# distributed-information-bottleneck/distributed-information-bottleneck.github.io

Measured on AMD Instinct MI355X. Metric: DIB train samples/sec (fwd+KL+bwd+Adam), higher is better.
Workload: dtype f32

## Files before the change

distributed-information-bottleneck.github.io_amd/csrc/dib_fused.h:

```cpp
#pragma once
#include "dib_common.h"
#include "dib_gemm.h"

struct DibFusedFwdArgs {
  const float* P;
  const int* row_idx; long long row0; int batch;
  const float* params;
  const long long* w_off;
  const long long* b_off;
  const int4* featmap;
  int n_blocks;
  int act;
  float* h1; float* h2; float* enc_out; float* U; float* kl_partial;
  unsigned long long* h2mask;
  unsigned long long* h1mask;
  int F; unsigned long long seed; unsigned step; int deterministic;
  const unsigned* step_dev;
};

template <int H1, int H2, int E>
struct DibFusedCfg {
  static constexpr int E2 = 2 * E;
  static constexpr int N3 = (E2 + 31) / 32 * 32;
  static constexpr int K1P = 36;
  static constexpr int P2 = H1 + 4, P3 = H2 + 4;
  static constexpr int W1_FLOATS = H1 * K1P, W2_FLOATS = H2 * P2, W3_FLOATS = N3 * P3;
  static constexpr int B_FLOATS = H1 + H2 + N3;
  static constexpr int PATCH = 32 * 36;
  static constexpr int LDS_FLOATS = W1_FLOATS + W2_FLOATS + W3_FLOATS + B_FLOATS + 8 * PATCH;
  static constexpr int T1 = H1 / 32, T2 = H2 / 32, T3 = N3 / 32;
};

typedef float dib_nt4 __attribute__((ext_vector_type(4)));

__device__ __forceinline__ int dib_crow(int r, int h) { return (r & 3) + 8 * (r >> 2) + 4 * h; }

__device__ __forceinline__ float dib_sigma(float lv) {
  return __builtin_amdgcn_exp2f(0.72134752044448170f * lv);
}

__device__ __forceinline__ float dib_neg_slope(int act) { return act == 1 ? 0.f : (act == 2 ? 0.2f : (act == 7 ? 0.1f : 1.f)); }
template <bool RELU>
__device__ __forceinline__ void dib_act_tile(float slope, dib_f32x16& v) {
#pragma unroll
  for (int r = 0; r < 16; ++r) v[r] = RELU ? fmaxf(v[r], 0.f) : fmaxf(v[r], 0.f) + slope * fminf(v[r], 0.f);
}

__device__ __forceinline__ int dib_patch_row(int lane, int pss) {
  return (lane >> 4) + 8 * ((lane >> 3) & 1) + 4 * (pss & 1) + 16 * (pss >> 1);
}

__device__ __forceinline__ int dib_store_idx(int lane) {
  return 4 * (((lane & 31) >> 2) >> 1) + (lane & 3);
}
__device__ __forceinline__ int dib_store_col(int lane) { return (dib_store_idx(lane) & 7) * 4; }
__device__ __forceinline__ int dib_store_row(int lane, int pss) {
  const int q = (lane & 31) >> 2;
  const int G = 2 * (lane >> 5) + ((0x96 >> q) & 1);
  return G + 4 * (pss & 1) + 16 * (pss >> 1) + 8 * (dib_store_idx(lane) >> 3);
}

__device__ __forceinline__ void dib_store_tile(float* __restrict__ patch, const dib_f32x16& c, float* __restrict__ dst,
                                               long long ld, int rows_valid, int lane) {
  const int m = lane & 31, h = lane >> 5;
#pragma unroll
  for (int g = 0; g < 4; ++g)
    *reinterpret_cast<float4*>(patch + m * 36 + 8 * g + 4 * h) = make_float4(c[4 * g], c[4 * g + 1], c[4 * g + 2], c[4 * g + 3]);
  __builtin_amdgcn_wave_barrier();
  const int cc = dib_store_col(lane);
  const int r0 = dib_store_row(lane, 0);
  const float* src = patch + r0 * 36 + cc;
  float4 v[4];
#pragma unroll
  for (int pss = 0; pss < 4; ++pss) v[pss] = *reinterpret_cast<const float4*>(src + (4 * (pss & 1) + 16 * (pss >> 1)) * 36);
  __builtin_amdgcn_wave_barrier();
  float* out = dst + (long long)r0 * ld + cc;
  if (rows_valid >= 32) {
#pragma unroll
    for (int pss = 0; pss < 4; ++pss)
      __builtin_nontemporal_store(dib_nt4{v[pss].x, v[pss].y, v[pss].z, v[pss].w},
                                  reinterpret_cast<dib_nt4*>(out + (long long)(4 * (pss & 1) + 16 * (pss >> 1)) * ld));
  } else {
#pragma unroll
    for (int pss = 0; pss < 4; ++pss)
      if (r0 + 4 * (pss & 1) + 16 * (pss >> 1) < rows_valid)
        *reinterpret_cast<float4*>(out + (long long)(4 * (pss & 1) + 16 * (pss >> 1)) * ld) = v[pss];
  }
}

template <int COUNT, typename LoadF, typename StoreF>
__device__ __forceinline__ void dib_stage_batched(int tid, LoadF load, StoreF store) {
  constexpr int ITERS = (COUNT + 511) / 512;
#pragma unroll
  for (int it0 = 0; it0 < ITERS; it0 += 8) {
    float v[8];
#pragma unroll
    for (int u = 0; u < 8; ++u) {
      const int i = tid + (it0 + u) * 512;
      v[u] = (it0 + u < ITERS && i < COUNT) ? load(i) : 0.f;
    }
#pragma unroll
    for (int u = 0; u < 8; ++u) {
      const int i = tid + (it0 + u) * 512;
      if (it0 + u < ITERS && i < COUNT) store(i, v[u]);
    }
  }
}

#ifdef DIB_FUSED_TIMING
__device__ long long dib_fused_dbg[16];
#define DIB_FT(i) do { __builtin_amdgcn_sched_barrier(0); const long long now_ = clock64(); tacc_[i] += now_ - tprev_; tprev_ = now_; \
                       __builtin_amdgcn_sched_barrier(0); } while (0)
#else
#define DIB_FT(i) do { } while (0)
#endif

template <int T>
__device__ __forceinline__ unsigned long long dib_sign_bits(const dib_f32x16 (&t)[T]) {
  static_assert(T <= 4, "one 64-bit mask word per lane");
  unsigned int word[2] = {0u, 0u};
#pragma unroll
  for (int w = 0; w < (T + 1) / 2; ++w)
#pragma unroll
    for (int idx = (16 * T - 32 * w - 1 < 31 ? 16 * T - 32 * w - 1 : 31); idx >= 0; --idx) {
      const int e = 32 * w + idx;
      int on;
      asm("v_med3_i32 %0, %1, 0, 1" : "=v"(on) : "v"(t[e >> 4][e & 15]));
      asm("v_lshl_or_b32 %0, %1, 1, %2" : "=v"(word[w]) : "v"(word[w]), "v"(on));
    }
  return ((unsigned long long)word[1] << 32) | word[0];
}
template <bool RELU>
__device__ __forceinline__ void dib_mask_tile(dib_f32x16& acc, unsigned long long bits, int jo, float slope) {
  const unsigned int word = (unsigned int)(bits >> (32 * ((16 * jo) >> 5)));
#pragma unroll
  for (int r = 0; r < 16; ++r) {
    const int keep = __builtin_amdgcn_sbfe(word, (16 * jo + r) & 31, 1);
    acc[r] = RELU ? __int_as_float(__float_as_int(acc[r]) & keep) : acc[r] * (keep ? 1.f : slope);
  }
}

template <int H1, int H2, int E, bool RELU>
__global__ void __launch_bounds__(512)
dib_fused_encoder_fwd_kernel(DibFusedFwdArgs a) {
  using C = DibFusedCfg<H1, H2, E>;
  extern __shared__ __attribute__((aligned(16))) float lds[];
  float* Wt1 = lds;
  float* Wt2 = Wt1 + C::W1_FLOATS;
  float* Wt3 = Wt2 + C::W2_FLOATS;
  float* Bs = Wt3 + C::W3_FLOATS;
  float* patch = Bs + C::B_FLOATS + (threadIdx.x >> 6) * C::PATCH;

  const int f = blockIdx.y;
  const int tid = threadIdx.x, lane = tid & 63, wave = tid >> 6;
  const int m = lane & 31, h = lane >> 5;
  const int4 fm = a.featmap[f];
  const int in_dim = fm.y;
  const int F = a.F;
  const float* Pf = a.P + (long long)fm.w * a.batch;

  {
    const float* W1 = a.params + a.w_off[0 * F + f];
    const float* W2 = a.params + a.w_off[1 * F + f];
    const float* W3 = a.params + a.w_off[2 * F + f];
    const float* b1 = a.params + a.b_off[0 * F + f];
    const float* b2 = a.params + a.b_off[1 * F + f];
    const float* b3 = a.params + a.b_off[2 * F + f];
    dib_stage_batched<H1 * 32>(tid, [&](int i) { const int k = i / H1; return (k < in_dim) ? W1[i] : 0.f; },
                               [&](int i, float v) { const int k = i / H1, n = i - k * H1; Wt1[n * C::K1P + k] = v; });
    dib_stage_batched<H1 * H2>(tid, [&](int i) { return W2[i]; },
                               [&](int i, float v) { const int k = i / H2, n = i - k * H2; Wt2[n * C::P2 + k] = v; });
    dib_stage_batched<H2 * C::N3>(tid, [&](int i) { const int k = i / C::N3, n = i - k * C::N3;
                                                    return (n < C::E2) ? W3[(long long)k * C::E2 + n] : 0.f; },
                                  [&](int i, float v) { const int k = i / C::N3, n = i - k * C::N3; Wt3[n * C::P3 + k] = v; });
    for (int i = tid; i < H1; i += 512) Bs[i] = b1[i];
    for (int i = tid; i < H2; i += 512) Bs[H1 + i] = b2[i];
    for (int i = tid; i < C::N3; i += 512) Bs[H1 + H2 + i] = (i < C::E2) ? b3[i] : 0.f;
  }
  __syncthreads();

  const int n_tiles = (a.batch + 255) / 256;
  const unsigned nstep = a.step_dev ? a.step_dev[0] : a.step;
  const float slope = dib_neg_slope(a.act);
  const int ksteps1 = 4 * ((in_dim + 7) / 8);
  float kl_acc = 0.f;

  auto load_p = [&](int tile, float (&dstp)[8]) {
    const int bb = min(tile * 256 + wave * 32 + m, a.batch - 1);
    const float* src = Pf + (long long)bb * in_dim;
#pragma unroll
    for (int r = 0; r < 8; ++r) {
      const int k = dib_crow(r, h);
      const float v = src[min(k, in_dim - 1)];
      dstp[r] = (k < in_dim) ? v : 0.f;
    }
  };
  float p[8], pn[8];
  if ((int)blockIdx.x < n_tiles) load_p(blockIdx.x, p);

#ifdef DIB_FUSED_TIMING
  long long tacc_[9] = {0, 0, 0, 0, 0, 0, 0, 0, 0};
  long long tprev_ = clock64();
  const long long tstart_ = tprev_;
  const long long wstart_ = wall_clock64();
  int ntl_ = 0;
#endif
  for (int tile = blockIdx.x; tile < n_tiles; tile += gridDim.x) {
#ifdef DIB_FUSED_TIMING
    ++ntl_;
#endif
    const int wrow0 = tile * 256 + wave * 32;
    const int rows_valid = min(32, a.batch - wrow0);
    const int b = wrow0 + m;
    const bool valid = b < a.batch;
    const long long grow = a.row_idx ? (long long)a.row_idx[valid ? b : 0] : a.row0 + b;
    {
      const int nt = tile + gridDim.x;
      load_p(nt < n_tiles ? nt : tile, pn);
    }

    dib_f32x16 h1[C::T1];
#pragma unroll
    for (int jo = 0; jo < C::T1; ++jo) {
      dib_f32x16 acc;
#pragma unroll
      for (int r = 0; r < 16; ++r) acc[r] = Bs[32 * jo + dib_crow(r, h)];
#pragma unroll
      for (int g = 0; g < 2; ++g) {
        if (4 * g < ksteps1) {
          const float4 w = *reinterpret_cast<const float4*>(Wt1 + (32 * jo + m) * C::K1P + 8 * g + 4 * h);
          acc = DIB_MFMA(w.x, p[4 * g + 0], acc);
          acc = DIB_MFMA(w.y, p[4 * g + 1], acc);
          acc = DIB_MFMA(w.z, p[4 * g + 2], acc);
          acc = DIB_MFMA(w.w, p[4 * g + 3], acc);
        }
      }
      dib_act_tile<RELU>(slope, acc);
      h1[jo] = acc;
    }
    DIB_FT(0);
    if (a.h1 != nullptr) {
      float* dst = a.h1 + ((long long)f * a.batch + wrow0) * H1;
#pragma unroll
      for (int jo = 0; jo < C::T1; ++jo) dib_store_tile(patch, h1[jo], dst + 32 * jo, H1, rows_valid, lane);
    }
    if (a.h1mask != nullptr && valid) a.h1mask[((long long)f * a.batch + b) * 2 + h] = dib_sign_bits<C::T1>(h1);
    DIB_FT(1);
    dib_f32x16 h2[C::T2];
    if constexpr (C::T2 % 2 == 0) {
#pragma unroll
    for (int jo = 0; jo < C::T2; jo += 2) {
      dib_f32x16 acc0, acc1;
#pragma unroll
      for (int r = 0; r < 16; ++r) { acc0[r] = Bs[H1 + 32 * jo + dib_crow(r, h)]; acc1[r] = Bs[H1 + 32 * jo + 32 + dib_crow(r, h)]; }
      const float* w0p = Wt2 + (32 * jo + m) * C::P2 + 4 * h;
      const float* w1p = w0p + 32 * C::P2;
      float4 wa = *reinterpret_cast<const float4*>(w0p), wb = *reinterpret_cast<const float4*>(w1p);
#pragma unroll
      for (int st = 0; st < 4 * C::T1; ++st) {
        const int ji = st >> 2, g = st & 3, sn = st + 1 < 4 * C::T1 ? st + 1 : st;
        const float4 wan = *reinterpret_cast<const float4*>(w0p + 8 * sn), wbn = *reinterpret_cast<const float4*>(w1p + 8 * sn);
        __builtin_amdgcn_sched_barrier(0);
        acc0 = DIB_MFMA(wa.x, h1[ji][4 * g + 0], acc0);
// ... 58 lines not shown
        const float4 wan = *reinterpret_cast<const float4*>(w0p + 8 * sn), wbn = *reinterpret_cast<const float4*>(w1p + 8 * sn);
        __builtin_amdgcn_sched_barrier(0);
        acc0 = DIB_MFMA(wa.x, h2[ji][4 * g + 0], acc0);
        acc1 = DIB_MFMA(wb.x, h2[ji][4 * g + 0], acc1);
        acc0 = DIB_MFMA(wa.y, h2[ji][4 * g + 1], acc0);
        acc1 = DIB_MFMA(wb.y, h2[ji][4 * g + 1], acc1);
        acc0 = DIB_MFMA(wa.z, h2[ji][4 * g + 2], acc0);
        acc1 = DIB_MFMA(wb.z, h2[ji][4 * g + 2], acc1);
        acc0 = DIB_MFMA(wa.w, h2[ji][4 * g + 3], acc0);
        acc1 = DIB_MFMA(wb.w, h2[ji][4 * g + 3], acc1);
        asm volatile("" : "+v"(acc0));
        asm volatile("" : "+v"(acc1));
        __builtin_amdgcn_sched_barrier(0);
        wa = wan; wb = wbn;
      }
      o[0] = acc0;
      o[1] = acc1;
    } else {
#pragma unroll
    for (int jo = 0; jo < C::T3; ++jo) {
      dib_f32x16 acc;
#pragma unroll
      for (int r = 0; r < 16; ++r) acc[r] = Bs[H1 + H2 + 32 * jo + dib_crow(r, h)];
#pragma unroll
      for (int ji = 0; ji < C::T2; ++ji) {
#pragma unroll
        for (int g = 0; g < 4; ++g) {
          const float4 w = *reinterpret_cast<const float4*>(Wt3 + (32 * jo + m) * C::P3 + 32 * ji + 8 * g + 4 * h);
          acc = DIB_MFMA(w.x, h2[ji][4 * g + 0], acc);
          acc = DIB_MFMA(w.y, h2[ji][4 * g + 1], acc);
          acc = DIB_MFMA(w.z, h2[ji][4 * g + 2], acc);
          acc = DIB_MFMA(w.w, h2[ji][4 * g + 3], acc);
        }
      }
      o[jo] = acc;
    }
    }
    DIB_FT(5);
    float klp = 0.f;
    float* eo = a.enc_out + ((long long)f * a.batch + b) * C::E2;
    float* up = a.U + (long long)b * ((long long)F * E) + (long long)f * E;
    constexpr int NG = E / 8;
    dib_f32x16 ut[(E >= 32) ? (E / 32) : 1];
#pragma unroll
    for (int gi = 0; gi < NG; ++gi) {
      const int t_mu = (E >= 32) ? (gi >> 2) : 0;
      const int g_mu = (E >= 32) ? (gi & 3) : gi;
      const int t_lv = (E >= 32) ? (t_mu + E / 32) : 0;
      const int g_lv = (E >= 32) ? g_mu : (gi + E / 8);
      const int e0 = 32 * t_mu + 8 * g_mu + 4 * h;
      float eps[4] = {0.f, 0.f, 0.f, 0.f};
      if (!a.deterministic) dib_eps4(a.seed, nstep, (uint32_t)grow, (uint32_t)f, (uint32_t)(e0 >> 2), eps);
      float4 mu = make_float4(o[t_mu][4 * g_mu], o[t_mu][4 * g_mu + 1], o[t_mu][4 * g_mu + 2], o[t_mu][4 * g_mu + 3]);
      float4 lv = make_float4(o[t_lv][4 * g_lv], o[t_lv][4 * g_lv + 1], o[t_lv][4 * g_lv + 2], o[t_lv][4 * g_lv + 3]);
      float4 u;
      const float4 sg = make_float4(dib_sigma(lv.x), dib_sigma(lv.y), dib_sigma(lv.z), dib_sigma(lv.w));
      u.x = mu.x + sg.x * eps[0];
      u.y = mu.y + sg.y * eps[1];
      u.z = mu.z + sg.z * eps[2];
      u.w = mu.w + sg.w * eps[3];
      ut[t_mu][4 * g_mu] = u.x; ut[t_mu][4 * g_mu + 1] = u.y; ut[t_mu][4 * g_mu + 2] = u.z; ut[t_mu][4 * g_mu + 3] = u.w;
      if (valid) {
        if (E < 32) {
          *reinterpret_cast<float4*>(eo + e0) = mu;
          *reinterpret_cast<float4*>(eo + E + e0) = lv;
          *reinterpret_cast<float4*>(up + e0) = u;
        }
        klp += 0.5f * ((mu.x * mu.x + sg.x * sg.x - lv.x - 1.f) + (mu.y * mu.y + sg.y * sg.y - lv.y - 1.f) +
                       (mu.z * mu.z + sg.z * sg.z - lv.z - 1.f) + (mu.w * mu.w + sg.w * sg.w - lv.w - 1.f));
      }
    }
    DIB_FT(6);
    if (E >= 32) {
      float* eo_w = a.enc_out + ((long long)f * a.batch + wrow0) * C::E2;
#pragma unroll
      for (int jo = 0; jo < C::T3; ++jo) dib_store_tile(patch, o[jo], eo_w + 32 * jo, C::E2, rows_valid, lane);
      float* u_w = a.U + (long long)wrow0 * ((long long)F * E) + (long long)f * E;
#pragma unroll
      for (int jo = 0; jo < ((E >= 32) ? (E / 32) : 1); ++jo)
        dib_store_tile(patch, ut[jo], u_w + 32 * jo, (long long)F * E, rows_valid, lane);
    }
    DIB_FT(7);
    kl_acc += dib_wave_sum(klp);
#pragma unroll
    for (int r = 0; r < 8; ++r) p[r] = pn[r];
    DIB_FT(8);
  }
#ifdef DIB_FUSED_TIMING
  if (blockIdx.x == 0 && blockIdx.y == 0 && tid == 0) {
    for (int i = 0; i < 9; ++i) dib_fused_dbg[i] = tacc_[i];
    dib_fused_dbg[9] = clock64() - tstart_;
    dib_fused_dbg[10] = ntl_;
    dib_fused_dbg[11] = wall_clock64() - wstart_;
  }
#endif
  if (lane == 0) a.kl_partial[((long long)blockIdx.x * 8 + wave) * F + f] = kl_acc;
}

typedef float dib_f32x4 __attribute__((ext_vector_type(4)));
#define DIB_MFMA16(a, b, c) __builtin_amdgcn_mfma_f32_16x16x4f32((a), (b), (c), 0, 0, 0)

struct DibFusedBwdArgs {
  const float* P; int batch;
  const float* params; const long long* w_off; const long long* b_off; const int4* featmap;
  int act;
  const unsigned long long* h1mask; const unsigned long long* h2mask;
  const float* enc_out; const float* U; const float* GU;
  float* dout; float* dh2;
  float* dw1_partial;
  const float* beta_dev; float inv_bg;
  int F;
};

template <int H1, int H2, int E>
struct DibFusedBwdCfg {
  static constexpr int E2 = 2 * E;
  static constexpr int N3 = (E2 + 31) / 32 * 32;
  static constexpr int P2 = H2 + 4, P3 = N3 + 4;
  static constexpr int W2_FLOATS = H1 * P2, W3_FLOATS = H2 * P3;
  static constexpr int PATCH = 32 * 36;
  static constexpr int LDS_FLOATS = W2_FLOATS + W3_FLOATS + 8 * PATCH;
  static constexpr int T1 = H1 / 32, T2 = H2 / 32, T3 = N3 / 32;
};

struct DibTile4 { float4 a, b, c, d; };
__device__ __forceinline__ DibTile4 dib_tile_gload(const float* __restrict__ src, long long ld, int rows_valid, int lane) {
  const int cc = (lane & 7) * 4;
  DibTile4 t;
  auto ld4 = [&](int pss) {
    const dib_nt4 v = __builtin_nontemporal_load(reinterpret_cast<const dib_nt4*>(src + (long long)min(dib_patch_row(lane, pss), rows_valid - 1) * ld + cc));
    return make_float4(v.x, v.y, v.z, v.w);
  };
  t.a = ld4(0); t.b = ld4(1); t.c = ld4(2); t.d = ld4(3);
  return t;
}
__device__ __forceinline__ dib_f32x16 dib_tile_to_frag(float* __restrict__ patch, const DibTile4 t, int lane) {
  const int cc = (lane & 7) * 4, m = lane & 31, h = lane >> 5;
  *reinterpret_cast<float4*>(patch + dib_patch_row(lane, 0) * 36 + cc) = t.a;
  *reinterpret_cast<float4*>(patch + dib_patch_row(lane, 1) * 36 + cc) = t.b;
  *reinterpret_cast<float4*>(patch + dib_patch_row(lane, 2) * 36 + cc) = t.c;
  *reinterpret_cast<float4*>(patch + dib_patch_row(lane, 3) * 36 + cc) = t.d;
  __builtin_amdgcn_wave_barrier();
  const float4 q0 = *reinterpret_cast<const float4*>(patch + m * 36 + 4 * h);
  const float4 q1 = *reinterpret_cast<const float4*>(patch + m * 36 + 8 + 4 * h);
  const float4 q2 = *reinterpret_cast<const float4*>(patch + m * 36 + 16 + 4 * h);
  const float4 q3 = *reinterpret_cast<const float4*>(patch + m * 36 + 24 + 4 * h);
  __builtin_amdgcn_wave_barrier();
  dib_f32x16 c;
  c[0] = q0.x; c[1] = q0.y; c[2] = q0.z; c[3] = q0.w; c[4] = q1.x; c[5] = q1.y; c[6] = q1.z; c[7] = q1.w;
  c[8] = q2.x; c[9] = q2.y; c[10] = q2.z; c[11] = q2.w; c[12] = q3.x; c[13] = q3.y; c[14] = q3.z; c[15] = q3.w;
  return c;
}

__device__ __forceinline__ int dib_dw1_row(int s8, int lg) { return s8 + 8 * lg; }

template <int H1, int H2, int E, bool RELU>
__global__ void __launch_bounds__(512)
dib_fused_encoder_bwd_kernel(DibFusedBwdArgs a) {
  static_assert(E % 32 == 0, "fused backward: embedding dimension must be a multiple of 32");
  static_assert(H1 / 32 <= 4 && H2 / 32 <= 4, "act' bit masks: one 64-bit word per (lane, layer)");
  using C = DibFusedBwdCfg<H1, H2, E>;
  extern __shared__ __attribute__((aligned(16))) float lds[];
  float* W2i = lds;
  float* W3i = W2i + C::W2_FLOATS;
  float* patch = W3i + C::W3_FLOATS + (threadIdx.x >> 6) * C::PATCH;

  const int f = blockIdx.y;
  const int tid = threadIdx.x, lane = tid & 63, wave = tid >> 6;
  const int m = lane & 31, h = lane >> 5;
  const int4 fm = a.featmap[f];
  const int in_dim = fm.y;
  const int F = a.F;
  const float* Pf = a.P + (long long)fm.w * a.batch;
  {
    const float* W2 = a.params + a.w_off[1 * F + f];
    const float* W3 = a.params + a.w_off[2 * F + f];
    dib_stage_batched<H1 * H2>(tid, [&](int i) { return W2[i]; },
                               [&](int i, float v) { const int k1 = i / H2, k2 = i - k1 * H2; W2i[k1 * C::P2 + k2] = v; });
    dib_stage_batched<H2 * C::N3>(tid, [&](int i) { const int k2 = i / C::N3, n = i - k2 * C::N3;
                                                    return (n < C::E2) ? W3[(long long)k2 * C::E2 + n] : 0.f; },
                                  [&](int i, float v) { const int k2 = i / C::N3, n = i - k2 * C::N3; W3i[k2 * C::P3 + n] = v; });
  }
  __syncthreads();

  const int n_tiles = (a.batch + 255) / 256;
  const float slope = dib_neg_slope(a.act);
  const float kb = a.beta_dev[0] * a.inv_bg;
  dib_f32x4 dw1[2 * C::T1];
#pragma unroll
  for (int t = 0; t < 2 * C::T1; ++t) dw1[t] = dib_f32x4{0.f, 0.f, 0.f, 0.f};
  const int l15 = lane & 15, lg = lane >> 4;

  for (int tile = blockIdx.x; tile < n_tiles; tile += gridDim.x) {
    const int wrow0 = tile * 256 + wave * 32;
    if (wrow0 >= a.batch) continue;
    const int rows_valid = min(32, a.batch - wrow0);
    const int b = min(wrow0 + m, a.batch - 1);
    const unsigned long long hbits = a.h2mask[((long long)f * a.batch + b) * 2 + h];
    const unsigned long long h1bits = a.h1mask[((long long)f * a.batch + b) * 2 + h];
    dib_f32x16 dout[C::T3];
    {
      const float* eo = a.enc_out + ((long long)f * a.batch + wrow0) * C::E2;
      const long long so = (long long)wrow0 * ((long long)F * E) + (long long)f * E;
#pragma unroll
      for (int t = 0; t < E / 32; ++t) {
        const DibTile4 vm = dib_tile_gload(eo + 32 * t, C::E2, rows_valid, lane);
        const DibTile4 vl = dib_tile_gload(eo + E + 32 * t, C::E2, rows_valid, lane);
        const DibTile4 vg = dib_tile_gload(a.GU + so + 32 * t, (long long)F * E, rows_valid, lane);
        const DibTile4 vu = dib_tile_gload(a.U + so + 32 * t, (long long)F * E, rows_valid, lane);
        const dib_f32x16 mu = dib_tile_to_frag(patch, vm, lane);
        const dib_f32x16 lv = dib_tile_to_frag(patch, vl, lane);
        const dib_f32x16 g = dib_tile_to_frag(patch, vg, lane);
        const dib_f32x16 u = dib_tile_to_frag(patch, vu, lane);
#pragma unroll
        for (int r = 0; r < 16; ++r) {
          const float s = dib_sigma(lv[r]);
          dout[t][r] = g[r] + kb * mu[r];
          dout[t + E / 32][r] = g[r] * (u[r] - mu[r]) * 0.5f + kb * 0.5f * (s * s - 1.f);
        }
      }
      float* dd = a.dout + ((long long)f * a.batch + wrow0) * C::E2;
#pragma unroll
      for (int t = 0; t < C::T3; ++t) dib_store_tile(patch, dout[t], dd + 32 * t, C::E2, rows_valid, lane);
    }

    float pa[8];
#pragma unroll
    for (int s8 = 0; s8 < 8; ++s8) {
      const int rl = dib_dw1_row(s8, lg);
      const float v = Pf[(long long)min(wrow0 + rl, a.batch - 1) * in_dim + min(l15, in_dim - 1)];
      pa[s8] = (rl < rows_valid) ? (l15 < in_dim ? v : (l15 == in_dim ? 1.f : 0.f)) : 0.f;
    }

    dib_f32x16 dh2[C::T2];
    {
      float* dg = a.dh2 + ((long long)f * a.batch + wrow0) * H2;
#pragma unroll
      for (int jo = 0; jo < C::T2; ++jo) {
        dib_f32x16 acc;
#pragma unroll
        for (int r = 0; r < 16; ++r) acc[r] = 0.f;
#pragma unroll
        for (int jt = 0; jt < C::T3; ++jt)
#pragma unroll
          for (int g = 0; g < 4; ++g) {
            const float4 w = *reinterpret_cast<const float4*>(W3i + (32 * jo + m) * C::P3 + 32 * jt + 8 * g + 4 * h);
            acc = DIB_MFMA(w.x, dout[jt][4 * g + 0], acc);
            acc = DIB_MFMA(w.y, dout[jt][4 * g + 1], acc);
            acc = DIB_MFMA(w.z, dout[jt][4 * g + 2], acc);
            acc = DIB_MFMA(w.w, dout[jt][4 * g + 3], acc);
          }
        dib_mask_tile<RELU>(acc, hbits, jo, slope);
        dh2[jo] = acc;
        dib_store_tile(patch, acc, dg + 32 * jo, H2, rows_valid, lane);
      }
    }

    {
#pragma unroll
      for (int jo = 0; jo < C::T1; ++jo) {
        dib_f32x16 acc;
#pragma unroll
        for (int r = 0; r < 16; ++r) acc[r] = 0.f;
#pragma unroll
        for (int jt = 0; jt < C::T2; ++jt)
#pragma unroll
          for (int g = 0; g < 4; ++g) {
            const float4 w = *reinterpret_cast<const float4*>(W2i + (32 * jo + m) * C::P2 + 32 * jt + 8 * g + 4 * h);
            acc = DIB_MFMA(w.x, dh2[jt][4 * g + 0], acc);
            acc = DIB_MFMA(w.y, dh2[jt][4 * g + 1], acc);
            acc = DIB_MFMA(w.z, dh2[jt][4 * g + 2], acc);
            acc = DIB_MFMA(w.w, dh2[jt][4 * g + 3], acc);
          }
        dib_mask_tile<RELU>(acc, h1bits, jo, slope);
#pragma unroll
        for (int g = 0; g < 4; ++g)
          *reinterpret_cast<float4*>(patch + m * 36 + 8 * g + 4 * h) =
              make_float4(acc[4 * g], acc[4 * g + 1], acc[4 * g + 2], acc[4 * g + 3]);
        __builtin_amdgcn_wave_barrier();
#pragma unroll
        for (int s8 = 0; s8 < 8; ++s8) {
          const int rl = dib_dw1_row(s8, lg);
          const float2 bb = *reinterpret_cast<const float2*>(patch + rl * 36 + 2 * l15);
          dw1[2 * jo] = DIB_MFMA16(pa[s8], bb.x, dw1[2 * jo]);
          dw1[2 * jo + 1] = DIB_MFMA16(pa[s8], bb.y, dw1[2 * jo + 1]);
        }
        __builtin_amdgcn_wave_barrier();
      }
    }
  }
  {
    float* dst = a.dw1_partial + (((long long)blockIdx.x * 8 + wave) * F + f) * (16ll * H1);
#pragma unroll
    for (int t = 0; t < 2 * C::T1; ++t)
#pragma unroll
      for (int r = 0; r < 4; ++r) {
        const int n = 32 * (t >> 1) + 2 * l15 + (t & 1);
        dst[(long long)(lg * 4 + r) * H1 + n] = dw1[t][r];
      }
  }
}

__global__ void __launch_bounds__(256)
dib_dw1_reduce_kernel(const float* __restrict__ partial, int nparts, int F, int H1, const long long* __restrict__ w_off,
                      const long long* __restrict__ b_off, const int4* __restrict__ featmap, float* __restrict__ grads) {
  const int f = blockIdx.x, k = blockIdx.y;
  const int in_dim = featmap[f].y;
  if (k > in_dim) return;
  const long long pstride = (long long)F * 16 * H1;
  for (int n = threadIdx.x; n < H1; n += 256) {
    const float* src = partial + ((long long)f * 16 + k) * H1 + n;
    float s = 0.f;
    int pz = 0;
    for (; pz + 8 <= nparts; pz += 8) {
      float v[8];
#pragma unroll
      for (int u = 0; u < 8; ++u) v[u] = src[(pz + u) * pstride];
#pragma unroll
      for (int u = 0; u < 8; ++u) s += v[u];
    }
    for (; pz < nparts; ++pz) s += src[pz * pstride];
    if (k < in_dim) grads[w_off[f] + (long long)k * H1 + n] = s;
    else grads[b_off[f] + n] = s;
  }
}
```

distributed-information-bottleneck.github.io_amd/csrc/host/encoder.h:

```cpp

template <int H1, int H2, int E, bool RELU>
static int launch_fused_fwd(const DibFusedFwdArgs& a, int gx, int F, hipStream_t st) {
  using C = DibFusedCfg<H1, H2, E>;
  const size_t lds = (size_t)C::LDS_FLOATS * sizeof(float);
  return launch_lds<&dib_fused_encoder_fwd_kernel<H1, H2, E, RELU>>(dim3(gx, F), dim3(512), lds, st, a);
}

static int fused_gx(const dib_layout* l, int batch) { return std::max(1, std::min(cdiv(batch, 256), std::max(1, 256 / l->F))); }

static bool fused_bwd_ok(const dib_layout* l) {
  if (!(l->fused_id == 0 || l->fused_id == 1)) return false;
  for (int f = 0; f < l->F; ++f)
    if (l->in_dim[f] > 15) return false;
  return true;
}

static bool use_small_enc(const dib_layout* l, int batch);
static dib_layout::H1Plan h1_recompute_plan(const dib_layout* l, const dib_layout::WsMap& m, const float* w, int batch) {
  dib_layout::H1Plan r;
  if (!knobs().wgrad_recompute_h1 || l->fused_id != 0 || !fused_bwd_ok(l) || l->h1_side.empty() || !l->dev_h1_side) return r;
  if (use_small_enc(l, batch)) return r;
  const GemmCall& c = l->enc_wgrad[1];
  WgradStreamPlan sp;
  if (!wgrad_stream_plan(l->table.data() + c.first, c, w + m.enc_h[0], w + m.g_enc_h[1], batch, m.nsplit, m.rows_per_split,
// ... 149 lines not shown
  float* w = (float*)ws;
  float* gt = wgrad_target(m, w, grads);
  const long long sstride = align_up(l->n_params, 4);
  int rc = DIB_OK;
  const bool small = use_small_enc(l, batch);
  const bool fused = small || fused_bwd_ok(l);
  const int LE = l->n_enc + 1;
  if (stages & 1) {
    if (small) {
      rc = small_encoder_bwd(l, m, w, batch, params, beta_dev, inv_global_batch, st);
    } else if (fused) {
      rc = fused_encoder_bwd(l, m, w, batch, params, beta_dev, inv_global_batch, st);
    } else {
      { ProfScope ps(kProfOther, (hipStream_t)stream);
      DIB_LAUNCH(dib_reparam_kl_bwd_kernel, dim3(m.kl_blocks, l->F), dim3(256), 0, st, w + m.enc_out, w + m.g_u,
                         w + m.U, w + m.dout, beta_dev, inv_global_batch, batch, l->F, l->E); }
      rc = (int)hipGetLastError();
    }
    if (rc) return rc;
  }
  for (int ly = LE - 1; ly >= 0; --ly) {
    const bool last = ly == LE - 1;
    const float* gout = last ? w + m.dout : w + m.g_enc_h[ly];
    const float* hin = ly == 0 ? w + m.P : w + m.enc_h[ly - 1];
    const bool wgrad_here = (last ? (stages & 2) : (stages & 1)) && !(fused && ly == 0);
    if (wgrad_here && ly == 1 && fused && !small) {
      const dib_layout::H1Plan plan = h1_plan_of(l, ws);
      if (plan.recompute) {
        const GemmCall& c = l->enc_wgrad[ly];
        rc = launch_wgrad_h1(plan.ch, l->act == 1, l->dev_groups, l->dev_h1_side, c, w + m.P, params, gout, gt, gt, batch, plan.nsplit,
                             plan.rows_per_split, sstride, st);
        if (rc == DIB_OK && m.nsplit > 1)
          rc = retire_stale_slabs(l, batch, l->table.data() + c.first, c.count, plan.nsplit, m.nsplit, gt, sstride, st);
        if (rc) return rc;
        continue;
      }
    }
    if (wgrad_here) {
      const bool halve = l->enc_wgrad[ly].max_n <= 64 && m.nsplit >= 32 && (m.nsplit % 2) == 0;
      rc = launch_gemm<2>(l, l->enc_wgrad[ly], hin, gout, gt, nullptr, nullptr, gt, batch, 0,
                          halve ? m.nsplit / 2 : m.nsplit, halve ? 2 * m.rows_per_split : m.rows_per_split, sstride, st,
                          m.nsplit);
      if (rc) return rc;
    }
    if ((stages & 1) && ly >= 1 && !fused) {
      rc = launch_gemm<1>(l, l->enc_dgrad[ly], gout, params, w + m.g_enc_h[ly - 1], nullptr, hin, nullptr, batch,
                          l->act, 1, 0, 0, st);
      if (rc) return rc;
    }
  }
  return DIB_OK;
}

extern "C" {

int dib_encoder_bank_fwd(dib_layout* l, const float* x, int64_t ldx, const int32_t* row_idx, int64_t row0, int batch,
                         const float* params, uint64_t seed, uint32_t step, int deterministic, void* ws,
                         dib_stream_t stream) {
  if (!l || !x || !params || !ws || batch <= 0) return DIB_E_ARG;
  if (!l->dev_groups) return DIB_E_WORKSPACE;
  hipStream_t st = (hipStream_t)stream;
  const auto m = l->map(batch);
  float* w = (float*)ws;
  { std::lock_guard<std::mutex> lk(l->wg_mu); l->fwd_training[ws] = !(deterministic & DIB_FWD_INFERENCE); }
  if (use_small_enc(l, batch)) {
    if (!(deterministic & DIB_FWD_INFERENCE)) h1_plan_record(l, ws, dib_layout::H1Plan());
    int rc = small_encoder_fwd(l, m, w, x, ldx, row_idx, row0, batch, params, seed, step, deterministic, st);
    if (rc || (deterministic & DIB_FWD_DEFER_SUMS)) return rc;
    ProfScope ps(kProfOther, st);
    DIB_LAUNCH(dib_colsum_partials_kernel, dim3(l->F), dim3(256), 0, st, w + m.kl_partial, small_tiles(batch), l->F,
                       w + m.step_out);
    return (int)hipGetLastError();
  }
  { ProfScope ps(kProfOther, (hipStream_t)stream);
  if ((long long)cdiv(l->sum_d, 64) * cdiv(batch, 64) >= 512)
    DIB_LAUNCH(dib_posenc_kernel<64>, dim3(cdiv(l->sum_d, 64), cdiv(batch, 64)), dim3(256), 0, st, x, (long long)ldx,
                       (const int*)row_idx, (long long)row0, batch, l->dev_colmap, l->sum_d, l->n_blocks, w + m.P);
  else
    DIB_LAUNCH(dib_posenc_kernel<16>, dim3(cdiv(l->sum_d, 64), cdiv(batch, 16)), dim3(256), 0, st, x, (long long)ldx,
                       (const int*)row_idx, (long long)row0, batch, l->dev_colmap, l->sum_d, l->n_blocks, w + m.P); }
  int rc = (int)hipGetLastError();
  if (rc) return rc;
  if (l->fused_id >= 0) {
    int gx = 1;
    rc = fused_encoder_fwd(l, m, w, x, ldx, row_idx, row0, batch, params, seed, step, deterministic, st, &gx);
    if (rc) return rc;
    if (deterministic & DIB_FWD_DEFER_SUMS) return DIB_OK;
    { ProfScope ps(kProfOther, (hipStream_t)stream);
    DIB_LAUNCH(dib_colsum_partials_kernel, dim3(l->F), dim3(256), 0, st, w + m.kl_partial, gx * 8, l->F,
                       w + m.step_out); }
    return (int)hipGetLastError();
  }
  rc = encoder_chain_fwd(l, m, w, batch, params, 0, l->F, st);
  if (rc) return rc;
  { ProfScope ps(kProfOther, (hipStream_t)stream);
  DIB_LAUNCH(dib_reparam_kl_fwd_kernel, dim3(m.kl_blocks, l->F), dim3(256), 0, st, w + m.enc_out, w + m.U,
                     w + m.kl_partial, (const int*)row_idx, (long long)row0, batch, l->F, l->E,
                     (unsigned long long)seed, (unsigned)step, deterministic & DIB_FWD_DETERMINISTIC, l->step_dev); }
  rc = (int)hipGetLastError();
  if (rc) return rc;
  if (deterministic & DIB_FWD_DEFER_SUMS) return DIB_OK;
  { ProfScope ps(kProfOther, (hipStream_t)stream);
  DIB_LAUNCH(dib_colsum_partials_kernel, dim3(l->F), dim3(256), 0, st, w + m.kl_partial, m.kl_blocks, l->F,
                     w + m.step_out); }
  return (int)hipGetLastError();
}

int dib_encoder_bank_bwd(dib_layout* l, int batch, const float* params, float* grads, const float* beta_dev,
                         float inv_global_batch, void* ws, dib_stream_t stream) {
  return encoder_bank_bwd_stages(l, batch, params, grads, beta_dev, inv_global_batch, 3, ws, stream);
}

int dib_encoder_bank_bwd_stage(dib_layout* l, int batch, const float* params, float* grads, const float* beta_dev,
                               float inv_global_batch, int stage, void* ws, dib_stream_t stream) {
  if (stage != 1 && stage != 2) return DIB_E_ARG;
  return encoder_bank_bwd_stages(l, batch, params, grads, beta_dev, inv_global_batch, stage, ws, stream);
}

int dib_workspace_h1_materialize(dib_layout* l, int batch, const float* params, void* ws, dib_stream_t stream) {
  if (!l || !params || !ws || batch <= 0 || l->n_enc < 1) return DIB_E_ARG;
  if (!l->dev_groups) return DIB_E_WORKSPACE;
  const auto m = l->map(batch);
  float* w = (float*)ws;
  return launch_gemm<0>(l, l->enc_fwd[0], w + m.P, params, w + m.enc_h[0], params, nullptr, nullptr, batch, l->act, 1, 0, 0,
                        (hipStream_t)stream);
}

int dib_encode_deterministic(dib_layout* l, int feature, const float* x_f, int n, const float* params, float* out,
                             void* ws, dib_stream_t stream) {
  if (!l || !x_f || !params || !out || !ws || n <= 0) return DIB_E_ARG;
  if (feature < 0 || feature >= l->F) return DIB_E_ARG;
  if (!l->dev_groups) return DIB_E_WORKSPACE;
  hipStream_t st = (hipStream_t)stream;
  const auto m = l->map(n);
  float* w = (float*)ws;
  const int d = l->dims[feature];
  { ProfScope ps(kProfOther, (hipStream_t)stream);
  DIB_LAUNCH(dib_posenc_kernel<64>, dim3(cdiv(d, 64), cdiv(n, 64)), dim3(256), 0, st, x_f, (long long)d,
                     (const int*)nullptr, 0ll, n, l->dev_colmap + l->x_off[feature], d, l->n_blocks, w + m.P); }
  int rc = (int)hipGetLastError();
  if (rc) return rc;
  rc = encoder_chain_fwd(l, m, w, n, params, feature, 1, st);
  if (rc) return rc;
  const int w2 = 2 * l->E;
  return (int)hipMemcpyAsync(out, w + m.enc_out + (int64_t)feature * n * w2, (size_t)n * w2 * sizeof(float),
                             hipMemcpyDeviceToDevice, st);
}

#ifdef DIB_FUSED_TIMING
int dib_fused_debug_read(long long* out16) {
  if (hipDeviceSynchronize() != hipSuccess) return DIB_E_ARG;
  return (int)hipMemcpyFromSymbol(out16, HIP_SYMBOL(dib_fused_dbg), 16 * sizeof(long long));
}
#endif

}
```

Measured before the change: 8.870 million.

## Prefetch next tile inputs and pair MFMA chains in fused encoder backward

Restructures the fused encoder backward loop so the next tile's masks, P values, GU/U and enc_out tiles are loaded into registers during the current tile's GEMMs (a software pipeline). The dout elementwise math is now done in row-major form before the LDS transpose, and dout is written with direct non-temporal global stores instead of going through the LDS patch. The dh2 and dh1 GEMMs process two output tiles at a time with double-buffered LDS weight reads and sched barriers. It also adds timing instrumentation behind a compile flag. The prefetch raises register pressure and may lower occupancy or cause spills.

```diff
diff --git a/distributed-information-bottleneck.github.io_amd/csrc/dib_fused.h b/distributed-information-bottleneck.github.io_amd/csrc/dib_fused.h
--- a/distributed-information-bottleneck.github.io_amd/csrc/dib_fused.h
+++ b/distributed-information-bottleneck.github.io_amd/csrc/dib_fused.h
@@ -109,6 +109,7 @@
 
 #ifdef DIB_FUSED_TIMING
 __device__ long long dib_fused_dbg[16];
+__device__ long long dib_fused_bwd_dbg[16];
 #define DIB_FT(i) do { __builtin_amdgcn_sched_barrier(0); const long long now_ = clock64(); tacc_[i] += now_ - tprev_; tprev_ = now_; \
                        __builtin_amdgcn_sched_barrier(0); } while (0)
 #else
@@ -473,6 +474,42 @@
   return c;
 }
 
+__device__ __forceinline__ void dib_tile_gstore(float* __restrict__ dst, long long ld, int rows_valid, int lane, const DibTile4& t) {
+  const int cc = (lane & 7) * 4;
+  const int r0 = dib_patch_row(lane, 0);
+  float* out = dst + (long long)r0 * ld + cc;
+  const float4 v[4] = {t.a, t.b, t.c, t.d};
+  if (rows_valid >= 32) {
+#pragma unroll
+    for (int pss = 0; pss < 4; ++pss)
+      __builtin_nontemporal_store(dib_nt4{v[pss].x, v[pss].y, v[pss].z, v[pss].w},
+                                  reinterpret_cast<dib_nt4*>(out + (long long)(4 * (pss & 1) + 16 * (pss >> 1)) * ld));
+  } else {
+#pragma unroll
+    for (int pss = 0; pss < 4; ++pss)
+      if (r0 + 4 * (pss & 1) + 16 * (pss >> 1) < rows_valid)
+        *reinterpret_cast<float4*>(out + (long long)(4 * (pss & 1) + 16 * (pss >> 1)) * ld) = v[pss];
+  }
+}
+__device__ __forceinline__ float dib_dmu(float mu, float g, float kb) { return fmaf(kb, mu, g); }
+__device__ __forceinline__ float dib_dlv(float mu, float lv, float g, float u, float kbh) {
+  const float s = dib_sigma(lv);
+  return fmaf(g * (u - mu), 0.5f, kbh * fmaf(s, s, -1.f));
+}
+__device__ __forceinline__ void dib_dout_rowmajor(const DibTile4& mu, const DibTile4& lv, const DibTile4& g, const DibTile4& u, float kb,
+                                                  DibTile4& dmu, DibTile4& dlv) {
+  const float kbh = kb * 0.5f;
+  auto one = [&](const float4& m4, const float4& l4, const float4& g4, const float4& u4, float4& dm, float4& dl) {
+    dm = make_float4(dib_dmu(m4.x, g4.x, kb), dib_dmu(m4.y, g4.y, kb), dib_dmu(m4.z, g4.z, kb), dib_dmu(m4.w, g4.w, kb));
+    dl = make_float4(dib_dlv(m4.x, l4.x, g4.x, u4.x, kbh), dib_dlv(m4.y, l4.y, g4.y, u4.y, kbh),
+                     dib_dlv(m4.z, l4.z, g4.z, u4.z, kbh), dib_dlv(m4.w, l4.w, g4.w, u4.w, kbh));
+  };
+  one(mu.a, lv.a, g.a, u.a, dmu.a, dlv.a);
+  one(mu.b, lv.b, g.b, u.b, dmu.b, dlv.b);
+  one(mu.c, lv.c, g.c, u.c, dmu.c, dlv.c);
+  one(mu.d, lv.d, g.d, u.d, dmu.d, dlv.d);
+}
+
 __device__ __forceinline__ int dib_dw1_row(int s8, int lg) { return s8 + 8 * lg; }
 
 template <int H1, int H2, int E, bool RELU>
@@ -512,50 +549,110 @@
   for (int t = 0; t < 2 * C::T1; ++t) dw1[t] = dib_f32x4{0.f, 0.f, 0.f, 0.f};
   const int l15 = lane & 15, lg = lane >> 4;
 
+  struct TileIn { unsigned long long hb, h1b; float pa[8]; DibTile4 vm[E / 32], vl[E / 32], vg[E / 32], vu[E / 32]; };
+  auto tile_row0 = [&](int tl) { return min(tl * 256 + wave * 32, a.batch - 1); };
+  auto load_early = [&](int tl, TileIn& in) {
+    const int w0 = tile_row0(tl), rv = min(32, a.batch - w0);
+    const int bq = min(w0 + m, a.batch - 1);
+    in.hb = a.h2mask[((long long)f * a.batch + bq) * 2 + h];
+    in.h1b = a.h1mask[((long long)f * a.batch + bq) * 2 + h];
+#pragma unroll
+    for (int s8 = 0; s8 < 8; ++s8)
+      in.pa[s8] = Pf[(long long)min(w0 + dib_dw1_row(s8, lg), a.batch - 1) * in_dim + min(l15, in_dim - 1)];
+    const long long so = (long long)w0 * ((long long)F * E) + (long long)f * E;
+#pragma unroll
+    for (int t = 0; t < E / 32; ++t) {
+      in.vg[t] = dib_tile_gload(a.GU + so + 32 * t, (long long)F * E, rv, lane);
+      in.vu[t] = dib_tile_gload(a.U + so + 32 * t, (long long)F * E, rv, lane);
+    }
+  };
+  auto load_late = [&](int tl, TileIn& in) {
+    const int w0 = tile_row0(tl), rv = min(32, a.batch - w0);
+    const float* eo = a.enc_out + ((long long)f * a.batch + w0) * C::E2;
+#pragma unroll
+    for (int t = 0; t < E / 32; ++t) {
+      in.vm[t] = dib_tile_gload(eo + 32 * t, C::E2, rv, lane);
+      in.vl[t] = dib_tile_gload(eo + E + 32 * t, C::E2, rv, lane);
+    }
+  };
+  TileIn cur;
+  if ((int)blockIdx.x < n_tiles) { load_late(blockIdx.x, cur); load_early(blockIdx.x, cur); }
+
+#ifdef DIB_FUSED_TIMING
+  long long tacc_[5] = {0, 0, 0, 0, 0};
+  long long tprev_ = clock64();
+  const long long tstart_ = tprev_;
+  const long long wstart_ = wall_clock64();
+  int ntl_ = 0;
+#endif
   for (int tile = blockIdx.x; tile < n_tiles; tile += gridDim.x) {
     const int wrow0 = tile * 256 + wave * 32;
     if (wrow0 >= a.batch) continue;
+#ifdef DIB_FUSED_TIMING
+    ++ntl_;
+#endif
     const int rows_valid = min(32, a.batch - wrow0);
-    const int b = min(wrow0 + m, a.batch - 1);
-    const unsigned long long hbits = a.h2mask[((long long)f * a.batch + b) * 2 + h];
-    const unsigned long long h1bits = a.h1mask[((long long)f * a.batch + b) * 2 + h];
+    const unsigned long long hbits = cur.hb, h1bits = cur.h1b;
     dib_f32x16 dout[C::T3];
     {
-      const float* eo = a.enc_out + ((long long)f * a.batch + wrow0) * C::E2;
-      const long long so = (long long)wrow0 * ((long long)F * E) + (long long)f * E;
+      float* dd = a.dout + ((long long)f * a.batch + wrow0) * C::E2;
 #pragma unroll
       for (int t = 0; t < E / 32; ++t) {
-        const DibTile4 vm = dib_tile_gload(eo + 32 * t, C::E2, rows_valid, lane);
-        const DibTile4 vl = dib_tile_gload(eo + E + 32 * t, C::E2, rows_valid, lane);
-        const DibTile4 vg = dib_tile_gload(a.GU + so + 32 * t, (long long)F * E, rows_valid, lane);
-        const DibTile4 vu = dib_tile_gload(a.U + so + 32 * t, (long long)F * E, rows_valid, lane);
-        const dib_f32x16 mu = dib_tile_to_frag(patch, vm, lane);
-        const dib_f32x16 lv = dib_tile_to_frag(patch, vl, lane);
-        const dib_f32x16 g = dib_tile_to_frag(patch, vg, lane);
-        const dib_f32x16 u = dib_tile_to_frag(patch, vu, lane);
-#pragma unroll
-        for (int r = 0; r < 16; ++r) {
-          const float s = dib_sigma(lv[r]);
-          dout[t][r] = g[r] + kb * mu[r];
-          dout[t + E / 32][r] = g[r] * (u[r] - mu[r]) * 0.5f + kb * 0.5f * (s * s - 1.f);
-        }
-      }
-      float* dd = a.dout + ((long long)f * a.batch + wrow0) * C::E2;
-#pragma unroll
-      for (int t = 0; t < C::T3; ++t) dib_store_tile(patch, dout[t], dd + 32 * t, C::E2, rows_valid, lane);
-    }
-
+        DibTile4 dm, dl;
+        dib_dout_rowmajor(cur.vm[t], cur.vl[t], cur.vg[t], cur.vu[t], kb, dm, dl);
+        dout[t] = dib_tile_to_frag(patch, dm, lane);
+        dout[t + E / 32] = dib_tile_to_frag(patch, dl, lane);
+        DIB_FT(0);
+        dib_tile_gstore(dd + 32 * t, C::E2, rows_valid, lane, dm);
+        dib_tile_gstore(dd + E + 32 * t, C::E2, rows_valid, lane, dl);
+        DIB_FT(1);
+      }
+    }
     float pa[8];
 #pragma unroll
-    for (int s8 = 0; s8 < 8; ++s8) {
-      const int rl = dib_dw1_row(s8, lg);
-      const float v = Pf[(long long)min(wrow0 + rl, a.batch - 1) * in_dim + min(l15, in_dim - 1)];
-      pa[s8] = (rl < rows_valid) ? (l15 < in_dim ? v : (l15 == in_dim ? 1.f : 0.f)) : 0.f;
-    }
+    for (int s8 = 0; s8 < 8; ++s8)
+      pa[s8] = (dib_dw1_row(s8, lg) < rows_valid) ? (l15 < in_dim ? cur.pa[s8] : (l15 == in_dim ? 1.f : 0.f)) : 0.f;
 
     dib_f32x16 dh2[C::T2];
     {
       float* dg = a.dh2 + ((long long)f * a.batch + wrow0) * H2;
+      if constexpr (C::T2 % 2 == 0) {
+#pragma unroll
+        for (int jo = 0; jo < C::T2; jo += 2) {
+          dib_f32x16 acc0, acc1;
+#pragma unroll
+          for (int r = 0; r < 16; ++r) { acc0[r] = 0.f; acc1[r] = 0.f; }
+          const float* w0p = W3i + (32 * jo + m) * C::P3 + 4 * h;
+          const float* w1p = w0p + 32 * C::P3;
+          float4 wa = *reinterpret_cast<const float4*>(w0p), wb = *reinterpret_cast<const float4*>(w1p);
+#pragma unroll
+          for (int st = 0; st < 4 * C::T3; ++st) {
+            const int jt = st >> 2, g = st & 3, sn = st + 1 < 4 * C::T3 ? st + 1 : st;
+            const float4 wan = *reinterpret_cast<const float4*>(w0p + 8 * sn), wbn = *reinterpret_cast<const float4*>(w1p + 8 * sn);
+            __builtin_amdgcn_sched_barrier(0);
+            acc0 = DIB_MFMA(wa.x, dout[jt][4 * g + 0], acc0);
+            acc1 = DIB_MFMA(wb.x, dout[jt][4 * g + 0], acc1);
+            acc0 = DIB_MFMA(wa.y, dout[jt][4 * g + 1], acc0);
+            acc1 = DIB_MFMA(wb.y, dout[jt][4 * g + 1], acc1);
+            acc0 = DIB_MFMA(wa.z, dout[jt][4 * g + 2], acc0);
+            acc1 = DIB_MFMA(wb.z, dout[jt][4 * g + 2], acc1);
+            acc0 = DIB_MFMA(wa.w, dout[jt][4 * g + 3], acc0);
+            acc1 = DIB_MFMA(wb.w, dout[jt][4 * g + 3], acc1);
+            asm volatile("" : "+v"(acc0));
+            asm volatile("" : "+v"(acc1));
+            __builtin_amdgcn_sched_barrier(0);
+            wa = wan; wb = wbn;
+          }
+          dib_mask_tile<RELU>(acc0, hbits, jo, slope);
+          dib_mask_tile<RELU>(acc1, hbits, jo + 1, slope);
+          dh2[jo] = acc0;
+          dh2[jo + 1] = acc1;
+          DIB_FT(2);
+          dib_store_tile(patch, acc0, dg + 32 * jo, H2, rows_valid, lane);
+          dib_store_tile(patch, acc1, dg + 32 * jo + 32, H2, rows_valid, lane);
+          DIB_FT(3);
+        }
+      } else {
 #pragma unroll
       for (int jo = 0; jo < C::T2; ++jo) {
         dib_f32x16 acc;
@@ -573,11 +670,66 @@
           }
         dib_mask_tile<RELU>(acc, hbits, jo, slope);
         dh2[jo] = acc;
+        DIB_FT(2);
         dib_store_tile(patch, acc, dg + 32 * jo, H2, rows_valid, lane);
-      }
-    }
-
+        DIB_FT(3);
+      }
+      }
+    }
+
+    TileIn nxt;
+    const int nt = tile + gridDim.x < n_tiles ? tile + gridDim.x : tile;
+    load_early(nt, nxt);
+    __builtin_amdgcn_sched_barrier(0);
     {
+      auto dw1_tile = [&](dib_f32x16& acc, int jo) {
+        dib_mask_tile<RELU>(acc, h1bits, jo, slope);
+#pragma unroll
+        for (int g = 0; g < 4; ++g)
+          *reinterpret_cast<float4*>(patch + m * 36 + 8 * g + 4 * h) =
+              make_float4(acc[4 * g], acc[4 * g + 1], acc[4 * g + 2], acc[4 * g + 3]);
+        __builtin_amdgcn_wave_barrier();
+#pragma unroll
+        for (int s8 = 0; s8 < 8; ++s8) {
+          const int rl = dib_dw1_row(s8, lg);
+          const float2 bb = *reinterpret_cast<const float2*>(patch + rl * 36 + 2 * l15);
+          dw1[2 * jo] = DIB_MFMA16(pa[s8], bb.x, dw1[2 * jo]);
+          dw1[2 * jo + 1] = DIB_MFMA16(pa[s8], bb.y, dw1[2 * jo + 1]);
+        }
+        __builtin_amdgcn_wave_barrier();
+      };
+      if constexpr (C::T1 % 2 == 0) {
+#pragma unroll
+        for (int jo = 0; jo < C::T1; jo += 2) {
+          dib_f32x16 acc0, acc1;
+#pragma unroll
+          for (int r = 0; r < 16; ++r) { acc0[r] = 0.f; acc1[r] = 0.f; }
+          const float* w0p = W2i + (32 * jo + m) * C::P2 + 4 * h;
+          const float* w1p = w0p + 32 * C::P2;
+          float4 wa = *reinterpret_cast<const float4*>(w0p), wb = *reinterpret_cast<const float4*>(w1p);
+#pragma unroll
+          for (int st = 0; st < 4 * C::T2; ++st) {
+            const int jt = st >> 2, g = st & 3, sn = st + 1 < 4 * C::T2 ? st + 1 : st;
+            const float4 wan = *reinterpret_cast<const float4*>(w0p + 8 * sn), wbn = *reinterpret_cast<const float4*>(w1p + 8 * sn);
+            __builtin_amdgcn_sched_barrier(0);
+            acc0 = DIB_MFMA(wa.x, dh2[jt][4 * g + 0], acc0);
+            acc1 = DIB_MFMA(wb.x, dh2[jt][4 * g + 0], acc1);
+            acc0 = DIB_MFMA(wa.y, dh2[jt][4 * g + 1], acc0);
+            acc1 = DIB_MFMA(wb.y, dh2[jt][4 * g + 1], acc1);
+            acc0 = DIB_MFMA(wa.z, dh2[jt][4 * g + 2], acc0);
+            acc1 = DIB_MFMA(wb.z, dh2[jt][4 * g + 2], acc1);
+            acc0 = DIB_MFMA(wa.w, dh2[jt][4 * g + 3], acc0);
+            acc1 = DIB_MFMA(wb.w, dh2[jt][4 * g + 3], acc1);
+            asm volatile("" : "+v"(acc0));
+            asm volatile("" : "+v"(acc1));
+            __builtin_amdgcn_sched_barrier(0);
+            wa = wan; wb = wbn;
+          }
+          if (jo == C::T1 - 2) { load_late(nt, nxt); __builtin_amdgcn_sched_barrier(0); }
+          dw1_tile(acc0, jo);
+          dw1_tile(acc1, jo + 1);
+        }
+      } else {
 #pragma unroll
       for (int jo = 0; jo < C::T1; ++jo) {
         dib_f32x16 acc;
@@ -593,23 +745,22 @@
             acc = DIB_MFMA(w.z, dh2[jt][4 * g + 2], acc);
             acc = DIB_MFMA(w.w, dh2[jt][4 * g + 3], acc);
           }
-        dib_mask_tile<RELU>(acc, h1bits, jo, slope);
-#pragma unroll
-        for (int g = 0; g < 4; ++g)
-          *reinterpret_cast<float4*>(patch + m * 36 + 8 * g + 4 * h) =
-              make_float4(acc[4 * g], acc[4 * g + 1], acc[4 * g + 2], acc[4 * g + 3]);
-        __builtin_amdgcn_wave_barrier();
-#pragma unroll
-        for (int s8 = 0; s8 < 8; ++s8) {
-          const int rl = dib_dw1_row(s8, lg);
-          const float2 bb = *reinterpret_cast<const float2*>(patch + rl * 36 + 2 * l15);
-          dw1[2 * jo] = DIB_MFMA16(pa[s8], bb.x, dw1[2 * jo]);
-          dw1[2 * jo + 1] = DIB_MFMA16(pa[s8], bb.y, dw1[2 * jo + 1]);
-        }
-        __builtin_amdgcn_wave_barrier();
-      }
-    }
-  }
+        if (jo == C::T1 - 1) { load_late(nt, nxt); __builtin_amdgcn_sched_barrier(0); }
+        dw1_tile(acc, jo);
+      }
+      }
+    }
+    DIB_FT(4);
+    cur = nxt;
+  }
+#ifdef DIB_FUSED_TIMING
+  if (blockIdx.x == 0 && blockIdx.y == 0 && tid == 0) {
+    for (int i = 0; i < 5; ++i) dib_fused_bwd_dbg[i] = tacc_[i];
+    dib_fused_bwd_dbg[9] = clock64() - tstart_;
+    dib_fused_bwd_dbg[10] = ntl_;
+    dib_fused_bwd_dbg[11] = wall_clock64() - wstart_;
+  }
+#endif
   {
     float* dst = a.dw1_partial + (((long long)blockIdx.x * 8 + wave) * F + f) * (16ll * H1);
 #pragma unroll
diff --git a/distributed-information-bottleneck.github.io_amd/csrc/host/encoder.h b/distributed-information-bottleneck.github.io_amd/csrc/host/encoder.h
--- a/distributed-information-bottleneck.github.io_amd/csrc/host/encoder.h
+++ b/distributed-information-bottleneck.github.io_amd/csrc/host/encoder.h
@@ -325,6 +325,10 @@
   if (hipDeviceSynchronize() != hipSuccess) return DIB_E_ARG;
   return (int)hipMemcpyFromSymbol(out16, HIP_SYMBOL(dib_fused_dbg), 16 * sizeof(long long));
 }
+int dib_fused_bwd_debug_read(long long* out16) {
+  if (hipDeviceSynchronize() != hipSuccess) return DIB_E_ARG;
+  return (int)hipMemcpyFromSymbol(out16, HIP_SYMBOL(dib_fused_bwd_dbg), 16 * sizeof(long long));
+}
 #endif
 
 }
```

Result: no change. 8.798 million (-0.8%).
